# scverse/squidpy

Hardware: AMD Instinct MI355X
Metric: nhood_enrichment permutations/sec (1e6 spots x 30 clusters) (higher is better)
Workload: dtype u8 labels / u32 counts / i64 moments

## Files before the change

### squidpy_amd/csrc/sqgr_nhood.hip

```cpp
#include "sqgr_shuffle.h"

#include <algorithm>
#include <cstdlib>
#include <type_traits>

namespace sqgr {

constexpr int COUNT_THREADS = 1024;

__global__ __launch_bounds__(256) void k_count_wide16(int64_t nnz, const int32_t* __restrict__ erow, const int32_t* __restrict__ indices,
                                                      const uint16_t* __restrict__ slab_all, int64_t n, int K,
                                                      uint32_t* __restrict__ partial_all) {
    const int64_t e = blockIdx.x * (int64_t)blockDim.x + threadIdx.x;
    if (e >= nnz) return;
    const uint16_t* slab = slab_all + (size_t)blockIdx.y * n * 16;
    uint32_t* dst = partial_all + (size_t)blockIdx.y * ((size_t)K * K * 16);
    const uint4* ra = reinterpret_cast<const uint4*>(slab + (size_t)erow[e] * 16);
    const uint4* rb = reinterpret_cast<const uint4*>(slab + (size_t)indices[e] * 16);
    const uint4 a0 = ra[0], a1 = ra[1], b0 = rb[0], b1 = rb[1];
    const uint32_t wa[8] = {a0.x, a0.y, a0.z, a0.w, a1.x, a1.y, a1.z, a1.w};
    const uint32_t wb[8] = {b0.x, b0.y, b0.z, b0.w, b1.x, b1.y, b1.z, b1.w};
#pragma unroll
    for (int b = 0; b < 16; ++b) {
        const uint32_t la = (wa[b >> 1] >> ((b & 1) * 16)) & 0xFFFFu, lb = (wb[b >> 1] >> ((b & 1) * 16)) & 0xFFFFu;
        atomicAdd(&dst[((size_t)la * K + lb) * 16 + b], 1u);
    }
}

template <int B>
__global__ __launch_bounds__(256) void k_transpose_labels(int64_t n, const uint8_t* __restrict__ lab, int64_t nperm_valid,
                                                          uint8_t* __restrict__ slab_all, int pw) {
    int64_t i = blockIdx.x * (int64_t)blockDim.x + threadIdx.x;
    if (i >= n) return;
    const int batch = blockIdx.y;
    uint32_t w[B / 4];
#pragma unroll
    for (int k = 0; k < B / 4; ++k) w[k] = 0;
#pragma unroll
    for (int b = 0; b < B; ++b) {
        int64_t p = (int64_t)batch * B + b;
        w[b >> 2] |= (p < nperm_valid ? (uint32_t)lab[(size_t)p * n + i] : 0u) << (8 * (b & 3));
    }
    if constexpr (B == 16) {
        slab_store16(slab_all + (size_t)batch * n * 16, n, i, pw, w[0], w[1], w[2], w[3]);
    } else {
        uint4* dst = reinterpret_cast<uint4*>(slab_all + ((size_t)batch * n + i) * B);
#pragma unroll
        for (int v = 0; v < B / 16; ++v) dst[v] = make_uint4(w[4 * v], w[4 * v + 1], w[4 * v + 2], w[4 * v + 3]);
    }
}

__device__ __forceinline__ int xcd_chunk(int b, int nblk) {
    if (nblk % 8 != 0) return b;
    return (b & 7) * (nblk >> 3) + (b >> 3);
}

// ... 570 lines not shown
    };
    __builtin_amdgcn_s_setprio(3);
    if (e0 < nnz) {
        if (uniform_block)
            sweep(std::false_type{});
        else
            sweep(std::true_type{});
    }
#ifndef SQGR_DEBUG_NO_FLUSH_WAIT
    asm volatile("s_waitcnt lgkmcnt(0)" ::: "memory");
#endif
    __syncthreads();
    if constexpr (CM != 0) {
        uint32_t* dst16 = partial_all + ((size_t)blockIdx.y * nchunks + chunk) * ((size_t)cells * 8) + (size_t)pass * hist_words;
        for (int i = tid; i < hist_words; i += COUNT_THREADS) dst16[i] = hist[i];
        return;
    }
    uint32_t* dst = partial_all + ((size_t)blockIdx.y * nchunks + chunk) * ((size_t)K * K * 16) + (size_t)pass * K * K * B + (size_t)a0 * K * B;
    const float inv_k = 1.0f / (float)K;
    for (int i = tid; i < hist_words; i += COUNT_THREADS) {
        uint32_t v = hist[i];
        if (SPLIT == 1 && add_transposed) {
            const int pair = i / B, b = i - pair * B;
            const int la = (int)(((float)pair + 0.5f) * inv_k), lb = pair - la * K;
            v += hist[(lb * K + la) * B + b];
        }
        dst[i] = v;
    }
}

__global__ __launch_bounds__(COUNT_THREADS) void k_count_global(int64_t nnz, const int32_t* __restrict__ erow,
                                                                const int32_t* __restrict__ indices,
                                                                const uint8_t* __restrict__ slab_all, int64_t n, int K,
                                                                int64_t edges_per_block, uint32_t* __restrict__ partial_all) {
    constexpr int B = 16;
    const int K2 = K * K;
    const int tid = threadIdx.x;
    const uint8_t* slab = slab_all + (size_t)blockIdx.y * n * B;
    uint32_t* dst = partial_all + (size_t)blockIdx.y * ((size_t)K2 * B);
    const int64_t e0 = (int64_t)blockIdx.x * edges_per_block;
    const int64_t e1 = min(nnz, e0 + edges_per_block);
    for (int64_t e = e0 + tid; e < e1; e += COUNT_THREADS) {
        const uint4 ra = *reinterpret_cast<const uint4*>(slab + (size_t)erow[e] * B);
        const uint4 rb = *reinterpret_cast<const uint4*>(slab + (size_t)indices[e] * B);
        const uint32_t wa[4] = {ra.x, ra.y, ra.z, ra.w}, wb[4] = {rb.x, rb.y, rb.z, rb.w};
#pragma unroll
        for (int b = 0; b < B; ++b) {
            const uint32_t pair = ((wa[b >> 2] >> (8 * (b & 3))) & 255u) * K + ((wb[b >> 2] >> (8 * (b & 3))) & 255u);
            atomicAdd(&dst[(size_t)pair * B + b], 1u);
        }
    }
}

__global__ __launch_bounds__(256) void k_reduce(const uint32_t* __restrict__ partial_all, int nblk, int nsum, int hist_words, int B, int pw,
                                                int K, int sym, const int64_t* __restrict__ shift, int64_t perm_batch0,
                                                int64_t perm_begin, int64_t perm_end, int64_t* __restrict__ acc_sum,
                                                uint64_t* __restrict__ acc_sq, uint32_t* __restrict__ perms_out) {
    __shared__ unsigned long long part[4][64];
    const int wl = threadIdx.x & 63, slice = threadIdx.x >> 6;
    const int j = blockIdx.x * 64 + wl;
    const int batch = blockIdx.y;
    const int K2 = K * K;
    int pair = 0, b = 0, jt = 0;
    if (j < hist_words) {
        const int plane = j / (K2 * pw), rem = j - plane * (K2 * pw);
        pair = rem / pw;
        b = plane * pw + (rem - pair * pw);
        if (sym & 4) {
            const int la = pair / K, lb = pair - la * K;
            jt = plane * (K2 * pw) + (lb * K + la) * pw + (rem - pair * pw);
        }
    }
    unsigned long long c = 0;
    if (j < hist_words) {
        const uint32_t* src = partial_all + (size_t)batch * nblk * hist_words;
        for (int k = slice; k < nsum; k += 4) {
            c += src[(size_t)k * hist_words + j];
            if (sym & 4) c += src[(size_t)k * hist_words + jt];
        }
    }
    part[slice][wl] = c;
    __syncthreads();
    if (slice != 0 || j >= hist_words) return;
    c = part[0][wl] + part[1][wl] + part[2][wl] + part[3][wl];
    if (sym & 2) c >>= 1;
    const int64_t p = perm_batch0 + (int64_t)batch * B + b;
    if (p >= perm_end || p < perm_begin) return;
    const int64_t d = (int64_t)c - shift[pair];
    const size_t slot = (size_t)batch * hist_words + j;
    acc_sum[slot] += d;
    acc_sq[slot] += (uint64_t)(d * d);
    if (perms_out) perms_out[(size_t)(p - perm_begin) * K2 + pair] = (uint32_t)c;
}

template <bool TRI, int PW>
__global__ __launch_bounds__(256) void k_reduce16(const uint32_t* __restrict__ partial_all, int nblk, int cells, int K, int doubled,
                                                  const int64_t* __restrict__ shift, int64_t perm_batch0, int64_t perm_begin, int64_t perm_end,
                                                  int64_t* __restrict__ acc_sum, uint64_t* __restrict__ acc_sq, uint32_t* __restrict__ perms_out) {
    const int cell = blockIdx.x * 256 + threadIdx.x;
    const int batch = blockIdx.y;
    if (cell >= cells) return;
    const int K2 = K * K;
    const size_t words = (size_t)cells * 8;
    uint32_t c[16];
#pragma unroll
    for (int b = 0; b < 16; ++b) c[b] = 0;
    const uint32_t* src = partial_all + (size_t)batch * nblk * words + (size_t)cell * (PW / 2);
#pragma unroll 2
    for (int k = 0; k < nblk; ++k, src += words) {
#pragma unroll
        for (int plane = 0; plane < 16 / PW; ++plane) {
            const uint32_t* q = src + (size_t)plane * cells * (PW / 2);
            uint32_t w[PW / 2];
            if constexpr (PW == 16) {
                const uint4 v0 = *reinterpret_cast<const uint4*>(q), v1 = *reinterpret_cast<const uint4*>(q + 4);
                w[0] = v0.x; w[1] = v0.y; w[2] = v0.z; w[3] = v0.w; w[4] = v1.x; w[5] = v1.y; w[6] = v1.z; w[7] = v1.w;
            } else if constexpr (PW == 8) {
                const uint4 v0 = *reinterpret_cast<const uint4*>(q);
                w[0] = v0.x; w[1] = v0.y; w[2] = v0.z; w[3] = v0.w;
            } else if constexpr (PW == 4) {
                const uint2 v0 = *reinterpret_cast<const uint2*>(q);
                w[0] = v0.x; w[1] = v0.y;
            } else {
                w[0] = *q;
            }
#pragma unroll
            for (int i = 0; i < PW / 2; ++i) {
                c[plane * PW + 2 * i] += w[i] & 0xffffu;
                c[plane * PW + 2 * i + 1] += w[i] >> 16;
            }
        }
    }
    int pa[2], npairs = 1;
    bool diag = false;
    if constexpr (TRI) {
        int hi = (int)((sqrtf(8.0f * (float)cell + 1.0f) - 1.0f) * 0.5f);
        while (hi * (hi + 1) / 2 > cell) --hi;
        while ((hi + 1) * (hi + 2) / 2 <= cell) ++hi;
        const int lo = cell - hi * (hi + 1) / 2;
        diag = lo == hi;
        npairs = diag ? 1 : 2;
        pa[0] = lo * K + hi;
        pa[1] = hi * K + lo;
    } else {
        pa[0] = pa[1] = cell;
    }
    const int64_t p0 = perm_batch0 + (int64_t)batch * 16;
    for (int t = 0; t < npairs; ++t) {
        const int64_t sh = shift[pa[t]];
        int64_t sum = 0;
        uint64_t sq = 0;
#pragma unroll
        for (int b = 0; b < 16; ++b) {
            const int64_t p = p0 + b;
            if (p >= perm_end || p < perm_begin) continue;
            uint32_t cnt = c[b];
            if constexpr (TRI) cnt = diag ? (doubled ? cnt : 2 * cnt) : (doubled ? cnt >> 1 : cnt);
            const int64_t d = (int64_t)cnt - sh;
            sum += d;
            sq += (uint64_t)(d * d);
            if (perms_out) perms_out[(size_t)(p - perm_begin) * K2 + pa[t]] = cnt;
        }
        const size_t slot = (size_t)batch * K2 + pa[t];
        acc_sum[slot] += sum;
        acc_sq[slot] += sq;
    }
}

__global__ __launch_bounds__(256) void k_finalize(const int64_t* __restrict__ acc_sum, const uint64_t* __restrict__ acc_sq, int nbatch,
                                                  int hist_words, int pw, int K2, int64_t* __restrict__ out_sum,
                                                  uint64_t* __restrict__ out_sq) {
    const int j = blockIdx.x * 256 + threadIdx.x;
    if (j >= hist_words) return;
    int64_t s = 0;
    uint64_t q = 0;
    for (int t = 0; t < nbatch; ++t) {
        s += acc_sum[(size_t)t * hist_words + j];
        q += acc_sq[(size_t)t * hist_words + j];
    }
    const int pair = (j % (K2 * pw)) / pw;
    atomicAdd(reinterpret_cast<unsigned long long*>(out_sum) + pair, (unsigned long long)s);
    atomicAdd(reinterpret_cast<unsigned long long*>(out_sq) + pair, (unsigned long long)q);
}

__global__ __launch_bounds__(256) void k_sum_chunks(uint32_t* __restrict__ partial_all, int nblk, int hist_words) {
    const int j = blockIdx.x * 256 + threadIdx.x;
    if (j >= hist_words) return;
    uint32_t* src = partial_all + (size_t)blockIdx.y * nblk * hist_words + j;
    uint32_t c = 0;
    for (int k = 0; k < nblk; ++k) c += src[(size_t)k * hist_words];
    src[0] = c;
}

template <bool WEIGHTED>
__global__ __launch_bounds__(256) void k_edge_pairs(int64_t nnz, const int32_t* __restrict__ erow,
                                                    const int32_t* __restrict__ indices, const double* __restrict__ data,
                                                    const int32_t* __restrict__ labels, int K,
                                                    unsigned long long* __restrict__ out_u64, double* __restrict__ out_f64) {
    int64_t e = blockIdx.x * (int64_t)blockDim.x + threadIdx.x;
    if (e >= nnz) return;
    int la = labels[erow[e]], lb = labels[indices[e]];
    if (la < 0 || lb < 0) return;
    if (WEIGHTED)
        atomicAdd(&out_f64[la * K + lb], data[e]);
    else
        atomicAdd(&out_u64[la * K + lb], 1ull);
}

template <int WAVES>
__global__ __launch_bounds__(WAVES * 64) void k_edge_weight_partials(int64_t nnz, const int32_t* __restrict__ erow,
                                                                      const int32_t* __restrict__ indices, const double* __restrict__ data,
                                                                      const int32_t* __restrict__ labels, int K, int64_t edges_per_wave,
                                                                      double* __restrict__ partials) {
    extern __shared__ double s_acc[];
    const int K2 = K * K, lane = threadIdx.x & 63, wave = threadIdx.x >> 6;
    double* acc = s_acc + (size_t)wave * K2;
    for (int c = lane; c < K2; c += 64) acc[c] = 0.0;
    __builtin_amdgcn_fence(__ATOMIC_ACQ_REL, "wavefront");
    const int64_t w = (int64_t)blockIdx.x * WAVES + wave;
    const int64_t e0 = w * edges_per_wave, e1 = e0 + edges_per_wave < nnz ? e0 + edges_per_wave : nnz;
    for (int64_t base = e0; base < e1; base += 64) {
        const int64_t e = base + lane;
        int cell = -1;
        double wt = 0.0;
        if (e < e1) {
            const int la = labels[erow[e]], lb = labels[indices[e]];
            if (la >= 0 && lb >= 0) {
                cell = la * K + lb;
                wt = data[e];
            }
        }
        unsigned long long todo = __ballot(cell >= 0);
        while (todo) {
// ... 87 lines not shown
    const double m = second ? mean[c] : 0.0;
    constexpr int U = 16;
    int64_t q = 0;
    for (; q + U <= count; q += U) {
        uint32_t v[U];
#pragma unroll
        for (int u = 0; u < U; ++u) v[u] = col[(size_t)(q + u) * K2];
#pragma unroll
        for (int u = 0; u < U; ++u) {
            if (second) {
                const double d = (double)v[u] - m;
                a += d * d;
            } else {
                a += (double)v[u];
            }
        }
    }
    for (; q < count; ++q) {
        if (second) {
            const double d = (double)col[(size_t)q * K2] - m;
            a += d * d;
        } else {
            a += (double)col[(size_t)q * K2];
        }
    }
    acc[c] = a;
}
__global__ __launch_bounds__(64) void k_numpy_chain_finish(double* __restrict__ v, int K2, double P, int op) {
    const int c = blockIdx.x * 64 + threadIdx.x;
    if (c >= K2) return;
    const double x = v[c] / P;
    v[c] = op ? sqrt(x) : x;
}

}

using namespace sqgr;

struct sqgr_nhood {
    sqgr_ctx* ctx = nullptr;
    const sqgr_graph* g = nullptr;
    int64_t n = 0;
    int K = 0, K2 = 0;
    LabelShuffler shuf;
    DevBuf<uint8_t> wcol;
    DevBuf<uint64_t> pcg_states;
    int B = 16;
    int nblk = 0;
    int nbatch = 0;
    DevBuf<uint32_t> keys;
    DevBuf<uint8_t> slab;
    hipEvent_t ev_shuffled[2] = {nullptr, nullptr}, ev_counted[2] = {nullptr, nullptr};
    ~sqgr_nhood() {
        for (int i = 0; i < 2; ++i) {
            if (ev_shuffled[i]) (void)hipEventDestroy(ev_shuffled[i]);
            if (ev_counted[i]) (void)hipEventDestroy(ev_counted[i]);
        }
    }
    size_t keys_stride() const { return (size_t)nbatch * key_words_per_row(B, shuf.n_libs); }
    bool wide() const { return shuf.wide(); }
    size_t slab_stride() const { return (size_t)nbatch * n * B * (wide() ? 2 : 1) + SEG_SLAB_PAD; }
    DevBuf<uint32_t> partial;
    DevBuf<int64_t> acc_sum;
    DevBuf<uint64_t> acc_sq;
    DevBuf<int64_t> shift, fin;
    sqgr_comm* comm = nullptr;
    DevBuf<uint32_t> perms_dev;
    DevBuf<uint8_t> stage;

    int hist_words() const { return K2 * B; }
    int pass_cap = 16;
    int cap() const {
        static const int env_cap = [] { const char* e = getenv("SQGR_COUNT_PASS_B"); return e ? std::max(atoi(e), 1) : 16; }();
        return std::min(pass_cap, env_cap);
    }
    int cm() const {
        static const bool off = [] { const char* e = getenv("SQGR_COUNT_C16"); return e && atoi(e) == 0; }();
        if (off || wide() || B != 16 || (size_t)K2 * 16 * 4 <= LDS_BUDGET || cap() < 2) return 0;
        const bool sym = g->sym_state == 1;
        const size_t c = sym ? (size_t)K * (K + 1) / 2 : (size_t)K2;
        if (c * 2 * 2 > LDS_BUDGET) return 0;
        return sym ? 2 : 1;
    }
    int cells() const { return cm() == 2 ? K * (K + 1) / 2 : K2; }
    int be() const {
        if (cm()) {
            for (int b : {16, 8, 4, 2})
                if ((size_t)cells() * b * 2 <= LDS_BUDGET && b <= cap()) return b;
        }
        for (int b : {16, 8, 4, 2, 1})
            if ((size_t)K2 * b * 4 <= LDS_BUDGET && b <= cap()) return b;
        if (!wide() && (size_t)((K + 1) / 2) * K * 4 <= LDS_BUDGET) return 1;
        return 0;
    }
    int split() const { return (B == 16 && !wide() && !cm() && be() == 1 && (size_t)K2 * 4 > LDS_BUDGET) ? 2 : 1; }
    int partial_w() const { return (B == 16 && !wide() && be() > 0 && be() < 16) ? be() : B; }
    bool lds_path() const { return !wide() && (B == 32 || be() > 0); }
    int passes() const { return (B == 16 && !wide() && be() > 0) ? (16 / be()) * split() : 1; }
    int plane_w() const { return (B == 16 && !wide() && be() > 0) ? be() : 16; }
    size_t part_words() const { return cm() ? (size_t)cells() * 8 : (size_t)hist_words(); }
    int acc_words() const { return cm() ? K2 : hist_words(); }
    int acc_pw() const { return cm() ? 1 : partial_w(); }
    uint32_t edge_step() const { return be() == 16 ? 1024u : (be() == 8 ? 2048u : 4096u); }
    int64_t list_edges() const {
        if (lds_path() && g->sym_state == 1) return g->n_half + g->n_self;
        if (lds_path() && B == 16 && be() == 16 && !cm() && g->split_state == 1) return g->n_mutual + g->n_oneway;
        return g->nnz;
    }
    bool columns_valid = false;
    int64_t chunk_cap(bool relaxed) const {
        if (!cm()) return 0;
        const uint32_t w = (g->sym_state == 1 && g->n_self > 0) ? 2u : 1u;
        if (relaxed && shuf.max_label_count > 0 && (int64_t)shuf.max_label_count * std::max<int64_t>(g->max_row_len, 1) * w <= 65535) return 0;
        return (int64_t)(65535u / w / edge_step()) * edge_step();
    }
    int blocks_base(int nb, bool relaxed = false) const {
        int want = nblk;
        if (want <= 0) {
            const int cus = ctx->cu_count > 0 ? ctx->cu_count : 256;
            const int64_t fill = (((int64_t)4 * cus) / std::max(nb * passes(), 1)) & ~(int64_t)7;
            want = (int)std::max<int64_t>(8, std::min<int64_t>(cus, fill));
        }
        if (const int64_t capn = chunk_cap(relaxed)) {
            const int64_t need = ceil_div(std::max<int64_t>(list_edges(), 1), capn);
            if (need > want) want = (int)(nblk > 0 ? need : ceil_div(need, 8) * 8);
        }
        return want;
    }
    bool seg_active = false;
    int seg_res_blocks(int nseg_blk) const {
        if (!seg_active || g->n_seg_res == 0) return 0;
        const int64_t per = std::max<int64_t>(ceil_div(std::max<int64_t>(g->n_seg_edges, 1), nseg_blk), 1024);
        return (int)std::min<int64_t>(nseg_blk, ceil_div(g->n_seg_res, per));
    }
    int blocks_for(int nb, bool relaxed = false) const {
        const int base = blocks_base(nb, relaxed);
        return base + seg_res_blocks(base);
    }
    int nblk_launch = 0;
    int sym_launch = 0;
    int partial_blocks(int nb) const { return lds_path() ? blocks_for(nb) : 1; }
    size_t partial_words() const {
        size_t m = 0;
        for (int nb = 1; nb <= nbatch; ++nb) m = std::max(m, (size_t)nb * partial_blocks(nb));
        return m * part_words();
    }
    int resolve_tuning();
    int ensure_workspace();
    int launch_shuffle(int nb, int buf, hipStream_t st, bool independent) const {
        return shuf.launch_shuffle_raw(B, nb, keys.p + (size_t)buf * keys_stride(), slab.p + (size_t)buf * slab_stride(), st, independent, plane_w());
    }
    int begin_run(const int64_t* shift_host);
    int finish_run(int local_rc, int64_t n_perms, int64_t* out_sum, uint64_t* out_sumsq, uint32_t* out_perms);
    int count_batches(int nb, int buf);
    int reduce_batches(int nb, int64_t perm_batch0, int64_t perm_begin, int64_t perm_end, uint32_t* perms_out_dev);
// ... 14 lines not shown
        if (hipMemGetInfo(&free_b, &total_b) == hipSuccess && n > 0) {
            const int64_t fit = (int64_t)(free_b / 4) / (2 * n * B);
            nbatch = (int)std::max<int64_t>(1, std::min<int64_t>(160, fit));
        }
    }
    seg_active = false;
    const char* env_seg = getenv("SQGR_COUNT_SEGMENTS");
    const int seg_mode = env_seg ? atoi(env_seg) : 1;
    if (seg_mode != 0) {
        const char* why = nullptr;
        if (wide() || B != 16) why = "32-wide label rows or more than 256 clusters";
        else if (be() != 16 || cm()) why = "the counters of 16 permutations do not fit LDS in 32 bits (more than 50 clusters)";
        else if (count_debug() != 0) why = "a probe variant is selected (SQGR_COUNT_DEBUG)";
        else {
            int rc = g->seg_coverage();
            if (rc == SQGR_OK && g->seg_state == 0 && (seg_mode == 2 || g->n_seg_edges * 10 >= g->n_half * 9)) rc = g->ensure_seg();
            if (rc != SQGR_OK) {
                if (seg_mode == 2) return rc;
                (void)hipGetLastError();
                why = "the segment list could not be built";
            } else if (g->seg_state == -1) {
                why = g->seg_why ? g->seg_why : "the graph has no segment list";
            } else if (seg_mode != 2 && g->n_seg_edges * 10 < g->n_half * 9) {
                why = "the segments cover less than 90 % of the half edges";
            } else if (g->seg_state != 1) {
                why = "the segment list could not be built";
            }
        }
        if (seg_mode == 2 && why) {
            set_error("SQGR_COUNT_SEGMENTS=2: the segment kernel does not take this plan: %s", why);
            return SQGR_ERR_UNSUPPORTED;
        }
        seg_active = !why;
    }
    return SQGR_OK;
}

int sqgr_nhood::ensure_workspace() {
    SQGR_TRY(resolve_tuning());
    SQGR_TRY(keys.ensure(2 * keys_stride()));
    SQGR_TRY(shuf.ensure_tab_workspace(B, nbatch));
    {
        const uint8_t* had = slab.p;
        const size_t had_n = slab.n;
        SQGR_TRY(slab.ensure(2 * slab_stride()));
        if (slab.p != had || slab.n != had_n)
            for (int i = 1; i <= 2; ++i) SQGR_HIP(hipMemsetAsync(slab.p + i * slab_stride() - SEG_SLAB_PAD, 0, SEG_SLAB_PAD, ctx->stream));
    }
    for (int i = 0; i < 2; ++i) {
        if (!ev_shuffled[i]) SQGR_HIP(hipEventCreateWithFlags(&ev_shuffled[i], hipEventDisableTiming));
        if (!ev_counted[i]) SQGR_HIP(hipEventCreateWithFlags(&ev_counted[i], hipEventDisableTiming));
    }
    SQGR_TRY(partial.ensure(partial_words()));
    SQGR_TRY(acc_sum.ensure((size_t)nbatch * acc_words()));
    SQGR_TRY(acc_sq.ensure((size_t)nbatch * acc_words()));
    SQGR_TRY(shift.ensure((size_t)K2));
    SQGR_TRY(fin.ensure((size_t)2 * K2));
    return SQGR_OK;
}

int sqgr_nhood::begin_run(const int64_t* shift_host) {
    hipStream_t st = ctx->stream;
    if (shift_host)
        SQGR_HIP(hipMemcpyAsync(shift.p, shift_host, (size_t)K2 * 8, hipMemcpyHostToDevice, st));
    else
        SQGR_HIP(hipMemsetAsync(shift.p, 0, (size_t)K2 * 8, st));
    SQGR_HIP(hipMemsetAsync(acc_sum.p, 0, (size_t)nbatch * acc_words() * 8, st));
    SQGR_HIP(hipMemsetAsync(acc_sq.p, 0, (size_t)nbatch * acc_words() * 8, st));
    return SQGR_OK;
}

int sqgr_nhood::finish_run(int local_rc, int64_t n_perms, int64_t* out_sum, uint64_t* out_sumsq, uint32_t* out_perms) {
    hipStream_t st = ctx->stream;
    auto finalize = [&]() -> int {
        const int hw = acc_words();
        LaunchTimer t(ctx, "nhood_finalize");
        SQGR_HIP(hipMemsetAsync(fin.p, 0, (size_t)2 * K2 * 8, st));
        k_finalize<<<(unsigned)ceil_div(hw, 256), 256, 0, st>>>(acc_sum.p, acc_sq.p, nbatch, hw, acc_pw(), K2, fin.p,
                                                               reinterpret_cast<uint64_t*>(fin.p + K2));
        SQGR_HIP(hipGetLastError());
        return SQGR_OK;
    };
    if (local_rc == SQGR_OK) local_rc = finalize();
    SQGR_TRY(comm_agree(comm, local_rc, st));
    SQGR_TRY(comm_allreduce_i64_dev(comm, fin.p, (size_t)2 * K2, false, st));
    SQGR_HIP(hipMemcpyAsync(out_sum, fin.p, (size_t)K2 * 8, hipMemcpyDeviceToHost, st));
    SQGR_HIP(hipMemcpyAsync(out_sumsq, fin.p + K2, (size_t)K2 * 8, hipMemcpyDeviceToHost, st));
    if (out_perms && n_perms > 0)
        SQGR_HIP(hipMemcpyAsync(out_perms, perms_dev.p, (size_t)n_perms * K2 * 4, hipMemcpyDeviceToHost, st));
    SQGR_HIP(hipStreamSynchronize(st));
    return SQGR_OK;
}

int sqgr_nhood::count_batches(int nb, int buf) {
    const uint8_t* slab_p = slab.p + (size_t)buf * slab_stride();
    const int64_t nnz = g->nnz;
    hipStream_t st = ctx->stream;
    const int hw = hist_words();
    const int nblk = blocks_for(nb, columns_valid);
    nblk_launch = lds_path() ? nblk : 1;
    sym_launch = 0;
    const int mode = cm();
    const int ncell = cells();
    if (nnz == 0) {
        SQGR_HIP(hipMemsetAsync(partial.p, 0, (size_t)nb * nblk_launch * part_words() * 4, st));
        return SQGR_OK;
    }
    if (seg_active) {
        const int nseg_blk = blocks_base(nb, columns_valid), nres_blk = seg_res_blocks(nseg_blk);
        nblk_launch = nseg_blk + nres_blk;
        const size_t lds = (size_t)hw * 4;
        const uint32_t nseg = (uint32_t)g->n_seg, nres = (uint32_t)g->n_seg_res;
        const uint32_t epb = (uint32_t)(ceil_div(ceil_div(std::max<int64_t>(nseg, 1), nseg_blk), SEG_ITER) * SEG_ITER);
        LaunchTimer t(ctx, "nhood_count_seg_half");
        if (nb < nbatch) SQGR_HIP(hipMemsetAsync(const_cast<uint8_t*>(slab_p) + (size_t)nb * n * 16, 0, SEG_SLAB_PAD, st));
        if (lds * 2 <= LDS_BUDGET) {
            SQGR_TRY(allow_lds(k_count_seg<8>, lds));
            k_count_seg<8><<<dim3(nseg_blk, nb), COUNT_THREADS, lds, st>>>(nseg, g->seg.p, slab_p, n, K, hw, epb, nblk_launch, partial.p);
        } else {
            SQGR_TRY(allow_lds(k_count_seg<4>, lds));
            k_count_seg<4><<<dim3(nseg_blk, nb), COUNT_THREADS, lds, st>>>(nseg, g->seg.p, slab_p, n, K, hw, epb, nblk_launch, partial.p);
        }
        if (nres_blk) {
            const uint32_t epb_r = (uint32_t)(ceil_div(ceil_div((int64_t)nres, nres_blk), 1024) * 1024);
            if (lds * 2 <= LDS_BUDGET) {
                SQGR_TRY(allow_lds((k_count<16, 8, false>), lds));
                k_count<16, 8, false><<<dim3(nres_blk, nb), COUNT_THREADS, lds, st>>>(nres, g->seg_res.p, slab_p, n, K, hw, epb_r, nres, 1, partial.p, nseg_blk);
            } else {
                SQGR_TRY(allow_lds((k_count<16, 4, false>), lds));
                k_count<16, 4, false><<<dim3(nres_blk, nb), COUNT_THREADS, lds, st>>>(nres, g->seg_res.p, slab_p, n, K, hw, epb_r, nres, 1, partial.p, nseg_blk);
            }
        }
        SQGR_HIP(hipGetLastError());
        return SQGR_OK;
    }
    if (wide()) {
        LaunchTimer t(ctx, "nhood_count_wide16");
        SQGR_HIP(hipMemsetAsync(partial.p, 0, (size_t)nb * hw * 4, st));
        k_count_wide16<<<dim3((unsigned)ceil_div(nnz, 256), nb), 256, 0, st>>>(nnz, g->erow.p, g->indices.p,
                                                                              reinterpret_cast<const uint16_t*>(slab_p), n, K, partial.p);
    } else if (lds_path() && B == 16 && be() < 16) {
        SQGR_TRY(g->ensure_half());
        const bool half = g->sym_state == 1;
// ... 99 lines not shown
        }
#define SQGR_COUNT(BB, MW, SELF) \
    k_count<BB, MW, SELF><<<grid, COUNT_THREADS, lds, st>>>(m, list, slab_p, n, K, hw, epb, self_begin, addt, partial.p)
        if (B == 32) {
            LaunchTimer t(ctx, half ? "nhood_count_b32_half" : "nhood_count_b32");
            if (self) {
                SQGR_TRY(allow_lds(k_count<32, 4, true>, lds));
                SQGR_COUNT(32, 4, true);
            } else {
                SQGR_TRY(allow_lds(k_count<32, 4, false>, lds));
                SQGR_COUNT(32, 4, false);
            }
        } else {
            LaunchTimer t(ctx, half ? "nhood_count_b16_half" : (split_list ? "nhood_count_b16_split" : "nhood_count_b16"));
            const int dbg = count_debug();
            if (dbg && lds * 2 <= LDS_BUDGET && !self) {
#define SQGR_COUNT_DBG(D) \
    case D: k_count<16, 8, false, D><<<grid, COUNT_THREADS, lds, st>>>(m, list, slab_p, n, K, hw, epb, self_begin, addt, partial.p); break
                switch (dbg) {
                    SQGR_COUNT_DBG(1); SQGR_COUNT_DBG(2); SQGR_COUNT_DBG(3); SQGR_COUNT_DBG(4); SQGR_COUNT_DBG(5); SQGR_COUNT_DBG(6);
                    default: k_count<16, 8, false, 7><<<grid, COUNT_THREADS, lds, st>>>(m, list, slab_p, n, K, hw, epb, self_begin, addt, partial.p);
                }
#undef SQGR_COUNT_DBG
            } else if (lds * 2 <= LDS_BUDGET) {
                if (self) SQGR_COUNT(16, 8, true); else SQGR_COUNT(16, 8, false);
            } else if (self) {
                SQGR_TRY(allow_lds(k_count<16, 4, true>, lds));
                SQGR_COUNT(16, 4, true);
            } else {
                SQGR_TRY(allow_lds(k_count<16, 4, false>, lds));
                SQGR_COUNT(16, 4, false);
            }
        }
#undef SQGR_COUNT
    } else {
        const int gblk = std::max(nblk, 64);
        const int64_t epb = ceil_div(nnz, gblk);
        LaunchTimer t(ctx, "nhood_count_global");
        SQGR_HIP(hipMemsetAsync(partial.p, 0, (size_t)nb * hw * 4, st));
        k_count_global<<<dim3(gblk, nb), COUNT_THREADS, 0, st>>>(nnz, g->erow.p, g->indices.p, slab_p, n, K, epb, partial.p);
    }
    SQGR_HIP(hipGetLastError());
    return SQGR_OK;
}

int sqgr_nhood::reduce_batches(int nb, int64_t perm_batch0, int64_t perm_begin, int64_t perm_end, uint32_t* perms_out_dev) {
    const int hw = hist_words();
    LaunchTimer t(ctx, "nhood_reduce");
    if (const int mode = cm()) {
        const int ncell = cells(), pw = partial_w();
        const dim3 grid((unsigned)ceil_div(ncell, 256), nb);
        const int dbl = (sym_launch & 2) ? 1 : 0;
#define SQGR_RED16(TRI, PW)                                                                                                                    \
    k_reduce16<TRI, PW><<<grid, 256, 0, ctx->stream>>>(partial.p, nblk_launch, ncell, K, dbl, shift.p, perm_batch0, perm_begin, perm_end, acc_sum.p, \
                                                       acc_sq.p, perms_out_dev)
#define SQGR_RED16_W(TRI)                                \
    switch (pw) {                                        \
        case 16: SQGR_RED16(TRI, 16); break;             \
        case 8: SQGR_RED16(TRI, 8); break;               \
        case 4: SQGR_RED16(TRI, 4); break;               \
        default: SQGR_RED16(TRI, 2); break;              \
    }
        if (mode == 2) { SQGR_RED16_W(true) } else { SQGR_RED16_W(false) }
#undef SQGR_RED16_W
#undef SQGR_RED16
        SQGR_HIP(hipGetLastError());
        return SQGR_OK;
    }
    int nsum = nblk_launch;
    if ((sym_launch & 4) && nblk_launch > 1) {
        k_sum_chunks<<<dim3((unsigned)ceil_div(hw, 256), nb), 256, 0, ctx->stream>>>(partial.p, nblk_launch, hw);
        nsum = 1;
    }
    k_reduce<<<dim3((unsigned)ceil_div(hw, 64), nb), 256, 0, ctx->stream>>>(partial.p, nblk_launch, nsum, hw, B, partial_w(), K, sym_launch, shift.p,
                                                                            perm_batch0, perm_begin, perm_end, acc_sum.p,
                                                                            acc_sq.p, perms_out_dev);
    SQGR_HIP(hipGetLastError());
    return SQGR_OK;
}

static int edge_pairs(sqgr_ctx* ctx, const sqgr_graph* g, const int32_t* labels, int32_t K, bool weighted, bool allow_negative,
                      unsigned long long* out_u64, double* out_f64) {
    SQGR_REQUIRE(ctx && g && labels, "ctx/graph/labels is NULL");
    SQGR_REQUIRE(g->ctx == ctx, "graph belongs to a different context");
    SQGR_REQUIRE(K >= 1, "K=%d", K);
    SQGR_TRY(check_labels(labels, g->n, K, allow_negative));
    SQGR_HIP(hipSetDevice(ctx->device));
    DevBuf<int32_t> dl;
    DevBuf<unsigned long long> du;
    DevBuf<double> dd;
    const size_t K2 = (size_t)K * K;
    SQGR_TRY(dl.alloc((size_t)g->n));
    SQGR_HIP(hipMemcpyAsync(dl.p, labels, (size_t)g->n * 4, hipMemcpyHostToDevice, ctx->stream));
    if (weighted) {
        SQGR_REQUIRE(g->has_data || g->nnz == 0, "graph was uploaded without edge data; weights unavailable");
        SQGR_TRY(dd.alloc(K2));
        SQGR_HIP(hipMemsetAsync(dd.p, 0, K2 * 8, ctx->stream));
    } else {
        SQGR_TRY(du.alloc(K2));
        SQGR_HIP(hipMemsetAsync(du.p, 0, K2 * 8, ctx->stream));
    }
    if (g->nnz > 0) {
        LaunchTimer t(ctx, "nhood_edge_pairs");
        unsigned grid = (unsigned)ceil_div(g->nnz, 256);
        if (weighted) {
            const size_t cell_bytes = K2 * 8;
            const int waves = cell_bytes * 4 <= 64 * 1024 ? 4 : (cell_bytes <= LDS_BUDGET ? 1 : 0);
            if (waves == 0) {
                k_edge_pairs<true><<<grid, 256, 0, ctx->stream>>>(g->nnz, g->erow.p, g->indices.p, g->data.p, dl.p, K, nullptr, dd.p);
            } else {
                const int64_t epw = std::max<int64_t>(64, ceil_div(ceil_div(g->nnz, 4096), 64) * 64);
                const int64_t nwaves = ceil_div(ceil_div(g->nnz, epw), waves) * waves;
                DevBuf<double> parts;
                SQGR_TRY(parts.alloc((size_t)nwaves * K2));
                if (waves == 4) {
                    k_edge_weight_partials<4><<<(unsigned)(nwaves / 4), 256, cell_bytes * 4, ctx->stream>>>(g->nnz, g->erow.p, g->indices.p, g->data.p,
                                                                                                           dl.p, K, epw, parts.p);
                } else {
                    SQGR_TRY(allow_lds(k_edge_weight_partials<1>, cell_bytes));
                    k_edge_weight_partials<1><<<(unsigned)nwaves, 64, cell_bytes, ctx->stream>>>(g->nnz, g->erow.p, g->indices.p, g->data.p, dl.p, K,
                                                                                                epw, parts.p);
                }
                k_sum_partials<<<(unsigned)ceil_div((int64_t)K2, 64), 64, 0, ctx->stream>>>(parts.p, nwaves, (int)K2, dd.p);
                SQGR_HIP(hipGetLastError());
                SQGR_HIP(hipStreamSynchronize(ctx->stream));
            }
        }
        else
            k_edge_pairs<false><<<grid, 256, 0, ctx->stream>>>(g->nnz, g->erow.p, g->indices.p, nullptr, dl.p, K, du.p, nullptr);
// ... 24 lines not shown
    if (weights) return edge_pairs(ctx, g, labels, K, true, true, nullptr, out);
    std::vector<unsigned long long> tmp((size_t)K * K);
    SQGR_TRY(edge_pairs(ctx, g, labels, K, false, true, tmp.data(), nullptr));
    for (size_t i = 0; i < tmp.size(); ++i) out[i] = (double)tmp[i];
    return SQGR_OK;
}

int sqgr_nhood_create(sqgr_ctx* ctx, const sqgr_graph* g, const int32_t* labels, int32_t K, const int32_t* lib_ids,
                      int32_t n_libs, sqgr_nhood** out_plan) {
    SQGR_REQUIRE(ctx && g && out_plan, "ctx/graph/out_plan is NULL");
    *out_plan = nullptr;
    SQGR_REQUIRE(g->ctx == ctx, "graph belongs to a different context");
    if (K > 4096) {
        set_error("K=%d > 4096 clusters is not supported by the batched permutation kernels", K);
        return SQGR_ERR_UNSUPPORTED;
    }
    if (K >= 2 && (g->n > (int64_t)1 << 27 || g->nnz > (int64_t)0xFFF00000u)) {
        set_error("graph too large for 32-bit slab offsets (n=%lld, nnz=%lld)", (long long)g->n, (long long)g->nnz);
        return SQGR_ERR_UNSUPPORTED;
    }
    sqgr_nhood* p = new sqgr_nhood();
    p->ctx = ctx;
    p->g = g;
    p->n = g->n;
    p->K = K;
    p->K2 = K * K;
    const int rc = LabelShuffler::create(ctx, g->n, labels, K, lib_ids, n_libs, &p->shuf);
    if (rc != SQGR_OK) {
        delete p;
        return rc;
    }
    *out_plan = p;
    return SQGR_OK;
}

int sqgr_nhood_destroy(sqgr_nhood* plan) {
    if (!plan) return SQGR_OK;
    (void)hipSetDevice(plan->ctx->device);
    delete plan;
    return SQGR_OK;
}

int sqgr_nhood_tune(sqgr_nhood* plan, int32_t perms_per_pass, int32_t blocks_per_batch, int32_t batches_per_launch) {
    SQGR_REQUIRE(plan, "plan is NULL");
    SQGR_REQUIRE(perms_per_pass == 0 || perms_per_pass == 16 || perms_per_pass == 32 || perms_per_pass == 8 || perms_per_pass == 4 ||
                     perms_per_pass == 2 || perms_per_pass == 1,
                 "perms_per_pass must be 0, 32, 16 (slab width) or 8, 4, 2, 1 (cap of the LDS pass width of a 16-wide slab)");
    SQGR_REQUIRE(blocks_per_batch >= 0 && blocks_per_batch <= 65535 && batches_per_launch >= 0 && batches_per_launch <= 1024,
                 "tuning value out of range");
    plan->B = perms_per_pass == 32 ? 32 : 16;
    plan->pass_cap = (perms_per_pass > 0 && perms_per_pass < 16) ? perms_per_pass : 16;
    plan->nblk = blocks_per_batch;
    plan->nbatch = batches_per_launch;
    plan->keys.release(); plan->slab.release(); plan->partial.release(); plan->acc_sum.release(); plan->acc_sq.release();
    return SQGR_OK;
}

int sqgr_nhood_run(sqgr_nhood* plan, uint64_t seed, int64_t perm_begin, int64_t perm_end, const int64_t* shift,
                   int64_t* out_sum, uint64_t* out_sumsq, uint32_t* out_perms) {
    SQGR_REQUIRE(plan && out_sum && out_sumsq, "plan/out_sum/out_sumsq is NULL");
    SQGR_REQUIRE(perm_begin >= 0 && perm_end >= perm_begin, "bad permutation range [%lld,%lld)", (long long)perm_begin,
                 (long long)perm_end);
    sqgr_nhood* p = plan;
    sqgr_ctx* ctx = p->ctx;
    SQGR_HIP(hipSetDevice(ctx->device));
    hipStream_t st = ctx->stream;
    const int K2 = p->K2;
    const int64_t nperm = perm_end - perm_begin;
    bool independent = false;
    SQGR_TRY(p->shuf.independent_mode(p->B, &independent));
    SQGR_REQUIRE(!independent || !p->shuf.mapped(), "SQGR_SHUFFLE_INDEPENDENT: no spot map");
    auto local = [&]() -> int {
    SQGR_TRY(p->ensure_workspace());
    const int B = p->B;
    const int64_t per_launch = (int64_t)p->nbatch * B;
    SQGR_TRY(p->begin_run(shift));
    if (out_perms && nperm > 0) SQGR_TRY(p->perms_dev.ensure((size_t)nperm * K2));
    const char* env_streams = getenv("SQGR_NHOOD_STREAMS");
    hipStream_t sa = (env_streams && atoi(env_streams) == 2) ? ctx->stream2 : st;
    int64_t grp = 0;
    for (int64_t p0 = perm_begin - perm_begin % FEISTEL_GROUP; p0 < perm_end; p0 += per_launch, ++grp) {
        const int64_t todo = (perm_end - p0 < per_launch) ? perm_end - p0 : per_launch;
        const int nb = (int)ceil_div(todo, B);
        const int buf = (sa != st) ? (int)(grp & 1) : 0;
        if (sa != st && grp >= 2) SQGR_HIP(hipStreamWaitEvent(sa, p->ev_counted[buf], 0));
        SQGR_TRY(p->shuf.keygen("nhood_keygen", seed, p0, nb, B, independent, p->keys.p + (size_t)buf * p->keys_stride(), sa));
        SQGR_TRY(p->launch_shuffle(nb, buf, sa, independent));
        SQGR_HIP(hipEventRecord(p->ev_shuffled[buf], sa));
        SQGR_HIP(hipStreamWaitEvent(st, p->ev_shuffled[buf], 0));
        p->columns_valid = p->shuf.has_labels;
        const int rc_count = p->count_batches(nb, buf);
        p->columns_valid = false;
        SQGR_TRY(rc_count);
        SQGR_TRY(p->reduce_batches(nb, p0, perm_begin, perm_end, out_perms ? p->perms_dev.p : nullptr));
        SQGR_HIP(hipEventRecord(p->ev_counted[buf], st));
    }
    return SQGR_OK;
    };
    return p->finish_run(local(), nperm, out_sum, out_sumsq, out_perms);
}

int sqgr_nhood_shuffled_labels(sqgr_nhood* plan, uint64_t seed, int64_t perm, uint8_t* out_labels) {
    SQGR_REQUIRE(plan && out_labels && perm >= 0, "plan/out_labels is NULL or perm < 0");
    SQGR_REQUIRE(plan->K <= 256, "sqgr_nhood_shuffled_labels returns uint8 labels: K=%d > 256", plan->K);
    SQGR_REQUIRE(!plan->shuf.mapped(), "a plan with a spot map (sqgr_nhood_set_spot_map) runs sqgr_nhood_run only");
    sqgr_nhood* p = plan;
    sqgr_ctx* ctx = p->ctx;
    SQGR_HIP(hipSetDevice(ctx->device));
    SQGR_TRY(p->ensure_workspace());
    hipStream_t st = ctx->stream;
    const int B = p->B;
    const int64_t perm_row = perm - perm % FEISTEL_GROUP;
    bool independent = false;
    SQGR_TRY(p->shuf.independent_mode(B, &independent));
    SQGR_TRY(p->shuf.keygen(nullptr, seed, perm_row, 1, B, independent, p->keys.p, st));
    SQGR_TRY(p->launch_shuffle(1, 0, st, independent));
    std::vector<uint8_t> rows((size_t)p->n * B);
    SQGR_HIP(hipMemcpyAsync(rows.data(), p->slab.p, rows.size(), hipMemcpyDeviceToHost, st));
    SQGR_HIP(hipStreamSynchronize(st));
    const int pw = p->plane_w(), slot = (int)(perm - perm_row);
    for (int64_t i = 0; i < p->n; ++i)
        out_labels[i] = pw == 16 || B != 16 ? rows[(size_t)i * B + (size_t)slot]
                                            : rows[(size_t)(slot / pw) * p->n * pw + (size_t)i * pw + (size_t)(slot % pw)];
    return SQGR_OK;
}

int sqgr_nhood_counts_batch(sqgr_ctx* ctx, const sqgr_graph* g, const uint8_t* labels, int64_t n_perms, int32_t K,
                            uint32_t* out_counts) {
    SQGR_REQUIRE(ctx && g && labels && out_counts, "ctx/graph/labels/out is NULL");
    SQGR_REQUIRE(n_perms >= 0, "n_perms < 0");
    SQGR_REQUIRE(K <= 256, "sqgr_nhood_counts_batch takes uint8 labels: K=%d > 256", K);
    const int64_t n = g->n;
    for (int64_t t = 0; t < n_perms * n; ++t)
        SQGR_REQUIRE(labels[t] < K, "labels[%lld]=%d outside [0,%d)", (long long)t, (int)labels[t], K);
    sqgr_nhood* p = nullptr;
    SQGR_TRY(sqgr_nhood_create(ctx, g, nullptr, K, nullptr, 0, &p));
    int rc = SQGR_OK;
    do {
        if ((rc = p->ensure_workspace()) != SQGR_OK) break;
        const int B = p->B, K2 = p->K2, hw = p->acc_words();
        const int64_t per_launch = (int64_t)p->nbatch * B;
        hipStream_t st = ctx->stream;
        if ((rc = p->stage.ensure((size_t)per_launch * n)) != SQGR_OK) break;
        if ((rc = p->perms_dev.ensure((size_t)(n_perms > 0 ? n_perms : 1) * K2)) != SQGR_OK) break;
        hipError_t e = hipMemsetAsync(p->shift.p, 0, (size_t)K2 * 8, st);
        if (e == hipSuccess) e = hipMemsetAsync(p->acc_sum.p, 0, (size_t)p->nbatch * hw * 8, st);
        if (e == hipSuccess) e = hipMemsetAsync(p->acc_sq.p, 0, (size_t)p->nbatch * hw * 8, st);
        for (int64_t p0 = 0; p0 < n_perms && e == hipSuccess && rc == SQGR_OK; p0 += per_launch) {
            const int64_t todo = (n_perms - p0 < per_launch) ? n_perms - p0 : per_launch;
            const int nb = (int)ceil_div(todo, B);
            e = hipMemcpyAsync(p->stage.p, labels + (size_t)p0 * n, (size_t)todo * n, hipMemcpyHostToDevice, st);
            if (e != hipSuccess) break;
            {
                LaunchTimer t(ctx, "nhood_transpose_labels");
                if (B == 32)
                    k_transpose_labels<32><<<dim3((unsigned)ceil_div(n, 256), nb), 256, 0, st>>>(n, p->stage.p, todo, p->slab.p, 16);
                else
                    k_transpose_labels<16><<<dim3((unsigned)ceil_div(n, 256), nb), 256, 0, st>>>(n, p->stage.p, todo, p->slab.p, p->plane_w());
            }
            if ((rc = p->count_batches(nb, 0)) != SQGR_OK) break;
            if ((rc = p->reduce_batches(nb, p0, 0, n_perms, p->perms_dev.p)) != SQGR_OK) break;
            e = hipStreamSynchronize(st);
        }
        if (rc != SQGR_OK) break;
        if (e == hipSuccess && n_perms > 0)
            e = hipMemcpyAsync(out_counts, p->perms_dev.p, (size_t)n_perms * K2 * 4, hipMemcpyDeviceToHost, st);
        if (e == hipSuccess) e = hipStreamSynchronize(st);
        if (e != hipSuccess) {
            set_error("nhood_counts_batch failed: %s", hipGetErrorString(e));
            rc = SQGR_ERR_HIP;
        }
    } while (0);
    sqgr_nhood_destroy(p);
    return rc;
}

static int run_pcg64_impl(sqgr_nhood* plan, const uint64_t* pcg_states, int64_t n_perms, const int64_t* shift, int64_t* out_sum,
                          uint64_t* out_sumsq, uint32_t* out_perms, bool keep_perms) {
    SQGR_REQUIRE(plan && pcg_states && out_sum && out_sumsq && n_perms >= 0, "null argument or n_perms < 0");
    SQGR_REQUIRE(!plan->shuf.mapped(), "a plan with a spot map (sqgr_nhood_set_spot_map) runs sqgr_nhood_run only: numpy's streams permute positions");
    sqgr_nhood* p = plan;
    keep_perms = keep_perms || out_perms != nullptr;
    SQGR_REQUIRE(p->shuf.has_labels, "plan was created without labels");
    sqgr_ctx* ctx = p->ctx;
    SQGR_HIP(hipSetDevice(ctx->device));
    hipStream_t st = ctx->stream;
    const int K2 = p->K2;
    LabelShuffler& sh = p->shuf;
    auto local = [&]() -> int {
    SQGR_TRY(p->ensure_workspace());
    const int B = p->B;
    const int64_t n = p->n;
    SQGR_TRY(p->begin_run(shift));
    if (keep_perms) SQGR_TRY(p->perms_dev.ensure((size_t)(n_perms + 1) * K2));
    if (p->wide()) {
        if (sh.has_libs) {
            set_error("K=%d > 256 clusters with library_key: numpy-stream shuffles are not available on the device", p->K);
            return SQGR_ERR_UNSUPPORTED;
        }
        size_t free_b = 0, total_b = 0;
// ... 172 lines not shown
```

Baseline: 1.330 million.

## Shrink nhood accumulators, add unsliced reduce path, and merge finalize buffers

The generic reduce kernel now sums the per-perm deltas across the pw lanes with wave shuffles, so the accumulators hold one slot per pair per plane instead of one per histogram word. It also gains an unsliced variant with unrolled loads for small chunk counts. Finalize is split across up to 16 batch slices, and the accumulator, sum-of-squares and result buffers are merged into one allocation. A single pinned host buffer replaces the two device-to-host copies, and the explicit finalize memset is dropped because the merged memset already zeroes it. The aim is less accumulator traffic, fewer memsets and copies, and more parallelism in reduce and finalize, at the cost of extra shuffles and a more intricate indexing scheme.

```diff
diff --git a/squidpy_amd/csrc/sqgr_nhood.hip b/squidpy_amd/csrc/sqgr_nhood.hip
--- a/squidpy_amd/csrc/sqgr_nhood.hip
+++ b/squidpy_amd/csrc/sqgr_nhood.hip
@@ -2,6 +2,7 @@
 
 #include <algorithm>
 #include <cstdlib>
+#include <cstring>
 #include <type_traits>
 
 namespace sqgr {
@@ -678,13 +679,15 @@
     }
 }
 
+constexpr int REDUCE_SLICED_FROM = 17;
+template <bool SLICED>
 __global__ __launch_bounds__(256) void k_reduce(const uint32_t* __restrict__ partial_all, int nblk, int nsum, int hist_words, int B, int pw,
                                                 int K, int sym, const int64_t* __restrict__ shift, int64_t perm_batch0,
                                                 int64_t perm_begin, int64_t perm_end, int64_t* __restrict__ acc_sum,
                                                 uint64_t* __restrict__ acc_sq, uint32_t* __restrict__ perms_out) {
-    __shared__ unsigned long long part[4][64];
-    const int wl = threadIdx.x & 63, slice = threadIdx.x >> 6;
-    const int j = blockIdx.x * 64 + wl;
+    __shared__ unsigned long long part[SLICED ? 4 : 1][64];
+    const int wl = threadIdx.x & 63, slice = SLICED ? threadIdx.x >> 6 : 0;
+    const int j = SLICED ? blockIdx.x * 64 + wl : blockIdx.x * 256 + (int)threadIdx.x;
     const int batch = blockIdx.y;
     const int K2 = K * K;
     int pair = 0, b = 0, jt = 0;
@@ -697,26 +700,50 @@
             jt = plane * (K2 * pw) + (lb * K + la) * pw + (rem - pair * pw);
         }
     }
+    const bool lead = slice == 0 && j < hist_words && (wl & (pw - 1)) == 0;
+    const size_t slot = (size_t)batch * (hist_words / pw) + (j < hist_words ? j / pw : 0);
+    const int64_t sh = slice == 0 ? shift[pair] : 0;
+    const int64_t had_sum = lead ? acc_sum[slot] : 0;
+    const uint64_t had_sq = lead ? acc_sq[slot] : 0;
     unsigned long long c = 0;
     if (j < hist_words) {
+        constexpr int STEP = SLICED ? 4 : 1, W = SLICED ? 4 : 8;
         const uint32_t* src = partial_all + (size_t)batch * nblk * hist_words;
-        for (int k = slice; k < nsum; k += 4) {
-            c += src[(size_t)k * hist_words + j];
-            if (sym & 4) c += src[(size_t)k * hist_words + jt];
-        }
-    }
-    part[slice][wl] = c;
-    __syncthreads();
-    if (slice != 0 || j >= hist_words) return;
-    c = part[0][wl] + part[1][wl] + part[2][wl] + part[3][wl];
+        auto walk = [&](int slot_j) {
+            const uint32_t* q = src + slot_j;
+            unsigned long long sum = 0;
+            for (int k = slice; k < nsum; k += W * STEP) {
+                uint32_t v[W];
+#pragma unroll
+                for (int u = 0; u < W; ++u) v[u] = q[(size_t)min(k + u * STEP, nsum - 1) * hist_words];
+#pragma unroll
+                for (int u = 0; u < W; ++u) sum += k + u * STEP < nsum ? v[u] : 0u;
+            }
+            return sum;
+        };
+        c = walk(j);
+        if (sym & 4) c += walk(jt);
+    }
+    if constexpr (SLICED) {
+        part[slice][wl] = c;
+        __syncthreads();
+        if (slice != 0) return;
+        c = part[0][wl] + part[1][wl] + part[2][wl] + part[3][wl];
+    }
     if (sym & 2) c >>= 1;
     const int64_t p = perm_batch0 + (int64_t)batch * B + b;
-    if (p >= perm_end || p < perm_begin) return;
-    const int64_t d = (int64_t)c - shift[pair];
-    const size_t slot = (size_t)batch * hist_words + j;
-    acc_sum[slot] += d;
-    acc_sq[slot] += (uint64_t)(d * d);
-    if (perms_out) perms_out[(size_t)(p - perm_begin) * K2 + pair] = (uint32_t)c;
+    const bool counted = j < hist_words && p < perm_end && p >= perm_begin;
+    const int64_t d = counted ? (int64_t)c - sh : 0;
+    if (counted && perms_out) perms_out[(size_t)(p - perm_begin) * K2 + pair] = (uint32_t)c;
+    int64_t s = d;
+    uint64_t q = (uint64_t)(d * d);
+    for (int o = 1; o < pw; o <<= 1) {
+        s += __shfl_xor(s, o);
+        q += __shfl_xor(q, o);
+    }
+    if (!lead) return;
+    acc_sum[slot] = had_sum + s;
+    acc_sq[slot] = had_sq + q;
 }
 
 template <bool TRI, int PW>
@@ -793,18 +820,18 @@
     }
 }
 
+constexpr int FINALIZE_SLICES = 16;
 __global__ __launch_bounds__(256) void k_finalize(const int64_t* __restrict__ acc_sum, const uint64_t* __restrict__ acc_sq, int nbatch,
-                                                  int hist_words, int pw, int K2, int64_t* __restrict__ out_sum,
-                                                  uint64_t* __restrict__ out_sq) {
+                                                  int acc_words, int K2, int64_t* __restrict__ out_sum, uint64_t* __restrict__ out_sq) {
     const int j = blockIdx.x * 256 + threadIdx.x;
-    if (j >= hist_words) return;
+    if (j >= acc_words) return;
     int64_t s = 0;
     uint64_t q = 0;
-    for (int t = 0; t < nbatch; ++t) {
-        s += acc_sum[(size_t)t * hist_words + j];
-        q += acc_sq[(size_t)t * hist_words + j];
-    }
-    const int pair = (j % (K2 * pw)) / pw;
+    for (int t = blockIdx.y; t < nbatch; t += gridDim.y) {
+        s += acc_sum[(size_t)t * acc_words + j];
+        q += acc_sq[(size_t)t * acc_words + j];
+    }
+    const int pair = j % K2;
     atomicAdd(reinterpret_cast<unsigned long long*>(out_sum) + pair, (unsigned long long)s);
     atomicAdd(reinterpret_cast<unsigned long long*>(out_sq) + pair, (unsigned long long)q);
 }
@@ -998,6 +1025,7 @@
     DevBuf<uint8_t> slab;
     hipEvent_t ev_shuffled[2] = {nullptr, nullptr}, ev_counted[2] = {nullptr, nullptr};
     ~sqgr_nhood() {
+        if (fin_host) (void)hipHostFree(fin_host);
         for (int i = 0; i < 2; ++i) {
             if (ev_shuffled[i]) (void)hipEventDestroy(ev_shuffled[i]);
             if (ev_counted[i]) (void)hipEventDestroy(ev_counted[i]);
@@ -1007,9 +1035,9 @@
     bool wide() const { return shuf.wide(); }
     size_t slab_stride() const { return (size_t)nbatch * n * B * (wide() ? 2 : 1) + SEG_SLAB_PAD; }
     DevBuf<uint32_t> partial;
-    DevBuf<int64_t> acc_sum;
-    DevBuf<uint64_t> acc_sq;
-    DevBuf<int64_t> shift, fin;
+    DevBuf<int64_t> acc;
+    DevBuf<int64_t> shift;
+    int64_t* fin_host = nullptr;
     sqgr_comm* comm = nullptr;
     DevBuf<uint32_t> perms_dev;
     DevBuf<uint8_t> stage;
@@ -1045,8 +1073,12 @@
     int passes() const { return (B == 16 && !wide() && be() > 0) ? (16 / be()) * split() : 1; }
     int plane_w() const { return (B == 16 && !wide() && be() > 0) ? be() : 16; }
     size_t part_words() const { return cm() ? (size_t)cells() * 8 : (size_t)hist_words(); }
-    int acc_words() const { return cm() ? K2 : hist_words(); }
-    int acc_pw() const { return cm() ? 1 : partial_w(); }
+    int acc_words() const { return cm() ? K2 : K2 * (B / partial_w()); }
+    size_t acc_slots() const { return (size_t)nbatch * acc_words(); }
+    size_t acc_total() const { return 2 * acc_slots() + (size_t)2 * K2; }
+    int64_t* acc_sum() const { return acc.p; }
+    uint64_t* acc_sq() const { return reinterpret_cast<uint64_t*>(acc.p + acc_slots()); }
+    int64_t* fin() const { return acc.p + 2 * acc_slots(); }
     uint32_t edge_step() const { return be() == 16 ? 1024u : (be() == 8 ? 2048u : 4096u); }
     int64_t list_edges() const {
         if (lds_path() && g->sym_state == 1) return g->n_half + g->n_self;
@@ -1167,10 +1199,9 @@
         if (!ev_counted[i]) SQGR_HIP(hipEventCreateWithFlags(&ev_counted[i], hipEventDisableTiming));
     }
     SQGR_TRY(partial.ensure(partial_words()));
-    SQGR_TRY(acc_sum.ensure((size_t)nbatch * acc_words()));
-    SQGR_TRY(acc_sq.ensure((size_t)nbatch * acc_words()));
+    SQGR_TRY(acc.ensure(acc_total()));
     SQGR_TRY(shift.ensure((size_t)K2));
-    SQGR_TRY(fin.ensure((size_t)2 * K2));
+    if (!fin_host) SQGR_HIP(hipHostMalloc(reinterpret_cast<void**>(&fin_host), (size_t)2 * K2 * 8, hipHostMallocDefault));
     return SQGR_OK;
 }
 
@@ -1180,8 +1211,7 @@
         SQGR_HIP(hipMemcpyAsync(shift.p, shift_host, (size_t)K2 * 8, hipMemcpyHostToDevice, st));
     else
         SQGR_HIP(hipMemsetAsync(shift.p, 0, (size_t)K2 * 8, st));
-    SQGR_HIP(hipMemsetAsync(acc_sum.p, 0, (size_t)nbatch * acc_words() * 8, st));
-    SQGR_HIP(hipMemsetAsync(acc_sq.p, 0, (size_t)nbatch * acc_words() * 8, st));
+    SQGR_HIP(hipMemsetAsync(acc.p, 0, acc_total() * 8, st));
     return SQGR_OK;
 }
 
@@ -1190,20 +1220,20 @@
     auto finalize = [&]() -> int {
         const int hw = acc_words();
         LaunchTimer t(ctx, "nhood_finalize");
-        SQGR_HIP(hipMemsetAsync(fin.p, 0, (size_t)2 * K2 * 8, st));
-        k_finalize<<<(unsigned)ceil_div(hw, 256), 256, 0, st>>>(acc_sum.p, acc_sq.p, nbatch, hw, acc_pw(), K2, fin.p,
-                                                               reinterpret_cast<uint64_t*>(fin.p + K2));
+        const dim3 grid((unsigned)ceil_div(hw, 256), (unsigned)std::min(nbatch, FINALIZE_SLICES));
+        k_finalize<<<grid, 256, 0, st>>>(acc_sum(), acc_sq(), nbatch, hw, K2, fin(), reinterpret_cast<uint64_t*>(fin() + K2));
         SQGR_HIP(hipGetLastError());
         return SQGR_OK;
     };
     if (local_rc == SQGR_OK) local_rc = finalize();
     SQGR_TRY(comm_agree(comm, local_rc, st));
-    SQGR_TRY(comm_allreduce_i64_dev(comm, fin.p, (size_t)2 * K2, false, st));
-    SQGR_HIP(hipMemcpyAsync(out_sum, fin.p, (size_t)K2 * 8, hipMemcpyDeviceToHost, st));
-    SQGR_HIP(hipMemcpyAsync(out_sumsq, fin.p + K2, (size_t)K2 * 8, hipMemcpyDeviceToHost, st));
+    SQGR_TRY(comm_allreduce_i64_dev(comm, fin(), (size_t)2 * K2, false, st));
+    SQGR_HIP(hipMemcpyAsync(fin_host, fin(), (size_t)2 * K2 * 8, hipMemcpyDeviceToHost, st));
     if (out_perms && n_perms > 0)
         SQGR_HIP(hipMemcpyAsync(out_perms, perms_dev.p, (size_t)n_perms * K2 * 4, hipMemcpyDeviceToHost, st));
     SQGR_HIP(hipStreamSynchronize(st));
+    memcpy(out_sum, fin_host, (size_t)K2 * 8);
+    memcpy(out_sumsq, fin_host + K2, (size_t)K2 * 8);
     return SQGR_OK;
 }
 
@@ -1409,8 +1439,8 @@
         const dim3 grid((unsigned)ceil_div(ncell, 256), nb);
         const int dbl = (sym_launch & 2) ? 1 : 0;
 #define SQGR_RED16(TRI, PW)                                                                                                                    \
-    k_reduce16<TRI, PW><<<grid, 256, 0, ctx->stream>>>(partial.p, nblk_launch, ncell, K, dbl, shift.p, perm_batch0, perm_begin, perm_end, acc_sum.p, \
-                                                       acc_sq.p, perms_out_dev)
+    k_reduce16<TRI, PW><<<grid, 256, 0, ctx->stream>>>(partial.p, nblk_launch, ncell, K, dbl, shift.p, perm_batch0, perm_begin, perm_end, acc_sum(), \
+                                                       acc_sq(), perms_out_dev)
 #define SQGR_RED16_W(TRI)                                \
     switch (pw) {                                        \
         case 16: SQGR_RED16(TRI, 16); break;             \
@@ -1429,9 +1459,14 @@
         k_sum_chunks<<<dim3((unsigned)ceil_div(hw, 256), nb), 256, 0, ctx->stream>>>(partial.p, nblk_launch, hw);
         nsum = 1;
     }
-    k_reduce<<<dim3((unsigned)ceil_div(hw, 64), nb), 256, 0, ctx->stream>>>(partial.p, nblk_launch, nsum, hw, B, partial_w(), K, sym_launch, shift.p,
-                                                                            perm_batch0, perm_begin, perm_end, acc_sum.p,
-                                                                            acc_sq.p, perms_out_dev);
+    if (nsum >= REDUCE_SLICED_FROM)
+        k_reduce<true><<<dim3((unsigned)ceil_div(hw, 64), nb), 256, 0, ctx->stream>>>(partial.p, nblk_launch, nsum, hw, B, partial_w(), K, sym_launch,
+                                                                                      shift.p, perm_batch0, perm_begin, perm_end, acc_sum(),
+                                                                                      acc_sq(), perms_out_dev);
+    else
+        k_reduce<false><<<dim3((unsigned)ceil_div(hw, 256), nb), 256, 0, ctx->stream>>>(partial.p, nblk_launch, nsum, hw, B, partial_w(), K, sym_launch,
+                                                                                        shift.p, perm_batch0, perm_begin, perm_end, acc_sum(),
+                                                                                        acc_sq(), perms_out_dev);
     SQGR_HIP(hipGetLastError());
     return SQGR_OK;
 }
@@ -1562,7 +1597,7 @@
     plan->pass_cap = (perms_per_pass > 0 && perms_per_pass < 16) ? perms_per_pass : 16;
     plan->nblk = blocks_per_batch;
     plan->nbatch = batches_per_launch;
-    plan->keys.release(); plan->slab.release(); plan->partial.release(); plan->acc_sum.release(); plan->acc_sq.release();
+    plan->keys.release(); plan->slab.release(); plan->partial.release(); plan->acc.release();
     return SQGR_OK;
 }
 
@@ -1648,14 +1683,13 @@
     int rc = SQGR_OK;
     do {
         if ((rc = p->ensure_workspace()) != SQGR_OK) break;
-        const int B = p->B, K2 = p->K2, hw = p->acc_words();
+        const int B = p->B, K2 = p->K2;
         const int64_t per_launch = (int64_t)p->nbatch * B;
         hipStream_t st = ctx->stream;
         if ((rc = p->stage.ensure((size_t)per_launch * n)) != SQGR_OK) break;
         if ((rc = p->perms_dev.ensure((size_t)(n_perms > 0 ? n_perms : 1) * K2)) != SQGR_OK) break;
         hipError_t e = hipMemsetAsync(p->shift.p, 0, (size_t)K2 * 8, st);
-        if (e == hipSuccess) e = hipMemsetAsync(p->acc_sum.p, 0, (size_t)p->nbatch * hw * 8, st);
-        if (e == hipSuccess) e = hipMemsetAsync(p->acc_sq.p, 0, (size_t)p->nbatch * hw * 8, st);
+        if (e == hipSuccess) e = hipMemsetAsync(p->acc.p, 0, p->acc_total() * 8, st);
         for (int64_t p0 = 0; p0 < n_perms && e == hipSuccess && rc == SQGR_OK; p0 += per_launch) {
             const int64_t todo = (n_perms - p0 < per_launch) ? n_perms - p0 : per_launch;
             const int nb = (int)ceil_div(todo, B);
```

New measurement: 1.363 million, median of 6. +2.5%, better.
